# yijingru/KG_Instance_Segmentation

Measured on AMD Instinct MI355X. Metric: imgs/s (train fwd+bwd) at 512x512, higher is better.
Workload: dtype forward: f32-tolerance, hi + lo f16 planes (22 significant bits), 3 MFMA products / backward: f16 single planes, 1 MFMA product; f16 MFMA, fp32 accumulate; 1 GPU; KGnet train step fwd(dec+seg)+4xDetectionLossAll+SEG_loss+bwd+Adam, batch 8/GPU 3x512x512, 300 boxes/img, full HIP path; precision_policy=fp32, global_batch=8, parallelism=dp1, loss_readback=every step (train.py:156), grad_overflow=False

## Files before the change

### include/kgnet_hip.h

```cpp
#ifndef KGNET_HIP_H
#define KGNET_HIP_H
#ifdef __cplusplus
extern "C" {
#endif

typedef struct kg_planes {
    int a_planes, a_pstride;
    int b_planes, b_pstride;
    int c_planes, c_pstride;
    int y_planes, y_pstride;
    int w_planes;
    int reserved_;
    const float* scale;
    const float* oscale;
} kg_planes_t;

int kg_rows_format(void);

const char* kg_last_error(void);
const char* kg_last_kernel(void);
int kg_version(void);
int kg_device_arch(char* out, int cap);
int kg_tr_probe(void* out_u16x256, void* stream);
int kg_f64_probe(const double* a, const double* b, double* out5n, int n, void* stream);
// ... 26 lines not shown
int kg_pack_weight_batch(const void* jobs, int njobs, int total_blocks, void* stream);
int kg_im2col_small(const void* x, void* out, int N, int H, int W, int OH, int OW, int KH, int KW, int stride, int pad, int cin,
                    int ldx, int Kpad, void* stream);
int kg_conv2d_wgrad(const void* x, const void* dy, float* dwp, const int* rowdesc, int M, int H, int W, int OH, int OW,
                    int ldx, int lddy, int Cin, int Cout, int cin_lim, int cout_lim, int KH, int KW, int stride, int pad,
                    int dil, int mode, int nsplit, long split_stride, const kg_planes_t* planes, void* stream);
int kg_conv2d_wgrad_halo(const void* x, const void* dy, float* dwp, int N, int H, int W, int ldx, int lddy, int Cin, int Cout,
                         int cin_lim, int cout_lim, int KS, int nsplit, long split_stride, const int* tiletab16, int ntiles,
                         float* dbp, const kg_planes_t* planes, void* stream);
int kg_bias_grad_final(const float* part, float* db, int nsplit, int C, int accumulate, void* stream);
int kg_wgrad_reduce(const float* part, float* grad_oihw, int Cout, int Cin, int KH, int KW, int nsplit, long split_stride,
                    int accumulate, void* stream);
int kg_wgrad_reduce_multi(const float* part, float* const* grads_oihw, const int* counts, int ngrads, int Cin, int KH, int KW,
                          int nsplit, long split_stride, int accumulate, void* stream);
int kg_wgrad_reduce_bias(const float* part, float* const* grads_oihw, const int* counts, int ngrads, int Cin, int KH, int KW,
                         int nsplit, long split_stride, int accumulate, const float* bias_part, float* db, int bias_C, void* stream);
int kg_wgrad_reduce_defer(int on);
int kg_wgrad_reduce_pending(void);
int kg_wgrad_reduce_flush(void* stream);
int kg_bias_grad(const void* dy, float* db, float* scratch, int scratch_floats, int M, int C, int ld, int accumulate,
                 void* stream);
int kg_set_wgrad_tr(int use_transpose_read);

int kg_img_pack(const float* img_nchw, void* out_rows8, int ldout, int N, int C, int H, int W, const kg_planes_t* planes, void* stream);
int kg_bn_stats_train(const void* x, int ldx, int M, int C, const float* gamma, const float* beta, float* running_mean,
                      float* running_var, float momentum, float eps, float* mean_out, float* invstd_out, float* scale,
                      float* shift, float* scratch, int scratch_floats, const kg_planes_t* planes, void* stream);
int kg_conv_stats_begin(float* part, long cap_floats);
int kg_conv_stats_end(int* nb);
int kg_bn_finalize_train(const float* part, int nb, int M, int C, const float* gamma, const float* beta, float* running_mean,
                         float* running_var, float momentum, float eps, float* mean_out, float* invstd_out, float* scale,
                         float* shift, void* stream);
int kg_bn_scale_shift_eval(int C, const float* gamma, const float* beta, const float* running_mean,
                           const float* running_var, float eps, float* scale, float* shift, void* stream);
int kg_bn_apply(const void* x, int ldx, const float* scale, const float* shift, const void* res, int ldres, void* y,
                int ldy, int M, int C, int relu, const kg_planes_t* planes, void* stream);
int kg_bn_bwd(const void* x, int ldx, const void* dy, int lddy, const float* gamma, const float* mean,
              const float* invstd, float* dgamma, float* dbeta, int accumulate, void* dx, int lddx, int M, int C,
              float* scratch, int scratch_floats, const float* parts, int nb_parts, const float* parts_scale,
              const kg_planes_t* planes, void* stream);
int kg_bn_bwd_frozen(const void* x, int ldx, const void* dy, int lddy, const float* scale, const float* running_mean,
                     const float* running_var, float eps, float* dgamma, float* dbeta, int accumulate, void* dx, int lddx,
                     int M, int C, float* scratch, int scratch_floats, const kg_planes_t* planes, void* stream);
int kg_conv_bstats_begin(float* part, long cap_floats, const void* x, int ldx, int x_planes, int x_pstride, const float* mean,
                         const float* invstd);
int kg_maxpool3s2_fwd(const void* x, int ldx, void* y, int ldy, void* argmax_u8, int N, int H, int W, int C, const kg_planes_t* planes, void* stream);
int kg_maxpool3s2_bwd(const void* x, int ldx, const void* dy, int lddy, void* dx, int lddx, const void* argmax_u8, int N, int H, int W, int C,
                      const kg_planes_t* planes, void* stream);
int kg_bilinear_fwd(const void* x, int ldx, void* y, int ldy, int N, int IH, int IW, int OH, int OW, int C,
                    const int* boxdesc, const int* row2box, long total_out_rows, const kg_planes_t* planes, void* stream);
int kg_bilinear_bwd(const void* dy, int lddy, void* dx, int lddx, int N, int IH, int IW, int OH, int OW, int C,
                    const int* boxdesc, const int* row2box, long total_in_rows, const void* mask, int ldmask,
                    const kg_planes_t* planes, void* stream);
int kg_add_rows(const void* a, int lda, const void* b, int ldb, const void* mask, int ldm, void* y, int ldy, long M,
                int C, const float* scale, const float* scale2, const kg_planes_t* planes, void* stream);
int kg_sigmoid_inplace(float* x, long n, void* stream);
int kg_grad_pack(const float* g_nchw, const float* prob, void* out_rows, int N, int C, int H, int W, int ld, int cpad,
                 const kg_planes_t* planes, void* stream);
int kg_grad_pack3(const float* g0_nchw, const float* g1_nchw, const float* g2_nchw, const float* prob0, void* out_rows, int N, int C0, int C1, int C2,
                  int H, int W, int ld, int pad0, int pad1, int pad2, const kg_planes_t* planes, void* stream);

int kg_detection_loss_fwd(const float* kp, const float* sh, const float* md, const float* gt, int N, int H, int W,
                          float kp_radius, const float* den_override, float* scratch, int scratch_floats, float* out8,
                          void* stream);
int kg_detection_loss_bwd(const float* kp, const float* sh, const float* md, const float* gt, int N, int H, int W,
                          float kp_radius, const float* fin8, const float* grad_out, float* g_kp, float* g_sh,
                          float* g_md, void* stream);
int kg_seg_loss(const float* prob, const void* tgt_u8, const int* patches, const void* pairs, int npatches, float* part,
                float* out1, const float* grad_out, float* gprob, void* stream);

int kg_postproc_timing_begin(void);
int kg_postproc_timing_end(float* ms4);
long kg_postproc_workspace_bytes(int H, int W, int peak_cap, int skel_cap);
int kg_postproc_scale(const float* kp, const float* soff, const float* mid, int H, int W, double thresh, void* ws,
                      long ws_bytes, int peak_cap, int skel_cap, double* skel, int* nskel, double* heat_out,
                      double* blur_out, int* peaks_out, double* peak_conf_out, int* npeaks_out, void* stream);
int kg_skeleton_boxes(const double* skel, const int* nskel, int skel_cap, double scale, int do_refine, double* boxes,
                      int* nbox, int box_cap, void* stream);
int kg_nms(const double* boxes, const int* nbox, int box_cap, double thresh, void* ws, long ws_bytes, double* out,
           int* nkeep, void* stream);

long kg_postproc_batch_workspace_bytes(int N, int H, int W, int peak_cap, int skel_cap);
int kg_postproc_batch(const float* kp, const float* soff, const float* mid, int N, int H, int W, double thresh, void* ws,
                      long ws_bytes, int peak_cap, int skel_cap, double* skel, int* nskel, void* stream);
int kg_skeleton_boxes_batch(int N, int nscales, const double* const* skel, const int* const* nskel, const int* skel_cap,
                            const double* scale, int do_refine, double* boxes, int* nbox, int box_cap, void* stream);
long kg_nms_batch_workspace_bytes(int N, int box_cap);
int kg_nms_batch(int N, const double* boxes, const int* nbox, int box_cap, double thresh, void* ws, long ws_bytes, double* out,
                 int* nkeep, void* stream);

int kg_gt_maps(const float* kps, int n, int H, int W, float* out, void* stream);

int kg_sp_image(const void* imgs, int N, int H, int W, float* out, void* stream);
int kg_sp_warp_masks(const void* imgs, const int* inst_img, int ntot, int H, int W, void* out, int* box, void* stream);
int kg_sp_boxes(const void* imgs, int N, const int* box, int ntot, int kp_radius, int* counts, float* gtb, float* kp, int* keep,
                void* stream);

int kg_adam_step(const void* jobs, int njobs, int total_blocks, float beta1, float beta2, float eps, float step_size, float bc2_sqrt,
                 float weight_decay, void* stream);

int kg_host_crop_masks(const float* const* masks, const int* work, int nwork, int H, int W, unsigned char* out);
int kg_crop_masks(const void* masks, const int* work, int nwork, int H, int W, void* out, void* stream);
int kg_host_tile_table(const int* h, const int* w, const long* row0, int nb, int th, int tw, int* out, int cap);
int kg_host_bin_csr(const int* tab, int nb, int BS, int BY, int BX, int nbins, int* bin_start, int* bin_boxes, int cap);
int kg_host_match_boxes(const float* pb, int P, const float* gb, int G, int gstride, float thresh, int* pairs, int cap, int* count);

// ... 91 lines not shown
```

### kg_instance_segmentation_amd/_lib.py

```python
import ctypes
import os

_HERE = os.path.dirname(os.path.abspath(__file__))
LIB_PATH = os.environ.get("KG_LIB_PATH") or os.path.join(_HERE, "libkgnet_hip.so")
LIB_F16_PATH = os.environ.get("KG_LIB_F16_PATH") or os.path.join(os.path.dirname(LIB_PATH), "libkgnet_hip_f16.so")

c_int, c_long, c_float, c_double, c_void_p = ctypes.c_int, ctypes.c_long, ctypes.c_float, ctypes.c_double, ctypes.c_void_p
P = c_void_p

_SIGS = {
    "kg_version": [],
    "kg_rows_format": [],
    "kg_grad_scale": [P, P, P, c_int, c_int, P, P, P],
    "kg_scale_tensors": [P, c_int, c_int, P, P],
    "kg_rows_rescale": [P, c_int, c_long, c_int, c_int, P, P, P, P, P, P],
    "kg_rows_scale": [P, c_int, c_long, c_int, P, P, P, P],
    "kg_rows_scale_multi": [P, c_int, P, P, P],
    "kg_device_arch": [ctypes.c_char_p, c_int],
    "kg_tr_probe": [P, P],
    "kg_conv2d_igemm": [P, P, P, P, P, P, P, P] + [c_int] * 21 + [P, P],
    "kg_conv2d_halo": [P, P, P, P, P, P, P] + [c_int] * 15 + [P, c_int, c_int, P, P],
    "kg_conv1x1": [P, P, P, P, P, P, c_long] + [c_int] * 8 + [P],
    "kg_conv3x3_c64": [P, P, P, P, P, P] + [c_int] * 11 + [P, c_int, P],
    "kg_conv3x3_ws": [P, P, P, P] + [c_int] * 7 + [P, c_int, P, P],
    "kg_pack_weight": [P, P] + [c_int] * 11 + [P],
    "kg_pack_weight_rows": [P, P] + [c_int] * 6 + [P, c_int, c_int, c_int, c_int, P],
    "kg_pack_weight_batch": [P, c_int, c_int, P],
    "kg_pack_weight_narrow": [P, P] + [c_int] * 9 + [P],
    "kg_conv7_narrow": [P, P, P, P] + [c_int] * 11 + [P],
    "kg_im2col_small": [P, P] + [c_int] * 12 + [P],
    "kg_conv2d_halo_heads2": [P, P, P, P, P, P, P] + [c_int] * 7 + [P, P],
    "kg_set_wgrad_tr": [c_int],
    "kg_conv2d_wgrad": [P, P, P, P] + [c_int] * 18 + [c_long, P, P],
    "kg_conv2d_wgrad_halo": [P, P, P] + [c_int] * 11 + [c_long, P, c_int, P, P, P],
    "kg_bias_grad_final": [P, P, c_int, c_int, c_int, P],
    "kg_wgrad_reduce": [P, P, c_int, c_int, c_int, c_int, c_int, c_long, c_int, P],
    "kg_wgrad_reduce_multi": [P, P, P, c_int, c_int, c_int, c_int, c_int, c_long, c_int, P],
    "kg_wgrad_reduce_bias": [P, P, P, c_int, c_int, c_int, c_int, c_int, c_long, c_int, P, P, c_int, P],
    "kg_wgrad_reduce_defer": [c_int],
    "kg_wgrad_reduce_pending": [],
    "kg_wgrad_reduce_flush": [P],
    "kg_bias_grad": [P, P, P, c_int, c_int, c_int, c_int, c_int, P],
    "kg_img_pack": [P, P, c_int, c_int, c_int, c_int, c_int, P, P],
    "kg_bn_stats_train": [P, c_int, c_int, c_int, P, P, P, P, c_float, c_float, P, P, P, P, P, c_int, P, P],
    "kg_bn_scale_shift_eval": [c_int, P, P, P, P, c_float, P, P, P],
    "kg_conv_stats_begin": [P, c_long],
    "kg_conv_bstats_begin": [P, c_long, P, c_int, c_int, c_int, P, P],
    "kg_conv_stats_end": [P],
    "kg_bn_finalize_train": [P, c_int, c_int, c_int, P, P, P, P, c_float, c_float, P, P, P, P, P],
    "kg_bn_apply": [P, c_int, P, P, P, c_int, P, c_int, c_int, c_int, c_int, P, P],
    "kg_bn_bwd": [P, c_int, P, c_int, P, P, P, P, P, c_int, P, c_int, c_int, c_int, P, c_int, P, c_int, P, P, P],
    "kg_bn_bwd_frozen": [P, c_int, P, c_int, P, P, P, c_float, P, P, c_int, P, c_int, c_int, c_int, P, c_int, P, P],
    "kg_maxpool3s2_fwd": [P, c_int, P, c_int, P, c_int, c_int, c_int, c_int, P, P],
    "kg_maxpool3s2_bwd": [P, c_int, P, c_int, P, c_int, P, c_int, c_int, c_int, c_int, P, P],
    "kg_bilinear_fwd": [P, c_int, P, c_int, c_int, c_int, c_int, c_int, c_int, c_int, P, P, c_long, P, P],
    "kg_bilinear_bwd": [P, c_int, P, c_int, c_int, c_int, c_int, c_int, c_int, c_int, P, P, c_long, P, c_int, P, P],
    "kg_add_rows": [P, c_int, P, c_int, P, c_int, P, c_int, c_long, c_int, P, P, P, P],
    "kg_detection_loss_fwd": [P, P, P, P, c_int, c_int, c_int, c_float, P, P, c_int, P, P],
    "kg_detection_loss_bwd": [P, P, P, P, c_int, c_int, c_int, c_float, P, P, P, P, P, P],
    "kg_seg_loss": [P, P, P, P, c_int, P, P, P, P, P],
    "kg_sigmoid_inplace": [P, c_long, P],
    "kg_grad_pack": [P, P, P, c_int, c_int, c_int, c_int, c_int, c_int, P, P],
    "kg_grad_pack3": [P, P, P, P, P] + [c_int] * 10 + [P, P],
    "kg_postproc_workspace_bytes": [c_int, c_int, c_int, c_int],
    "kg_postproc_scale": [P, P, P, c_int, c_int, c_double, P, c_long, c_int, c_int, P, P, P, P, P, P, P, P],
    "kg_postproc_timing_begin": [],
    "kg_postproc_timing_end": [P],
    "kg_skeleton_boxes": [P, P, c_int, c_double, c_int, P, P, c_int, P],
    "kg_nms": [P, P, c_int, c_double, P, c_long, P, P, P],
    "kg_postproc_batch_workspace_bytes": [c_int, c_int, c_int, c_int, c_int],
    "kg_postproc_batch": [P, P, P, c_int, c_int, c_int, c_double, P, c_long, c_int, c_int, P, P, P],
    "kg_skeleton_boxes_batch": [c_int, c_int, P, P, P, P, c_int, P, P, c_int, P],
    "kg_nms_batch_workspace_bytes": [c_int, c_int],
    "kg_nms_batch": [c_int, P, P, c_int, c_double, P, c_long, P, P, P],
    "kg_gt_maps": [P, c_int, c_int, c_int, P, P],
    "kg_sp_image": [P, c_int, c_int, c_int, P, P],
    "kg_sp_warp_masks": [P, P, c_int, c_int, c_int, P, P, P],
    "kg_sp_boxes": [P, c_int, P, c_int, c_int, P, P, P, P, P],
    "kg_adam_step": [P, c_int, c_int, c_float, c_float, c_float, c_float, c_float, c_float, P],
    "kg_host_crop_masks": [P, P, c_int, c_int, c_int, P],
    "kg_crop_masks": [P, P, c_int, c_int, c_int, P, P],
    "kg_host_match_boxes": [P, c_int, P, c_int, c_int, c_float, P, c_int, P],
    "kg_host_tile_table": [P, P, P, c_int, c_int, c_int, P, c_int],
    "kg_host_bin_csr": [P, c_int, c_int, c_int, c_int, c_int, P, P, c_int],
    "kg_mask_areas": [P, c_int, c_long, P, P],
    "kg_mask_inter_pairs": [P, P, P, c_int, c_long, P, P],
    "kg_mask_bits_ld": [c_int, c_int],
    "kg_mask_pack_bits": [P, c_int, c_int, c_int, c_int, P, c_long, P],
    "kg_mask_unpack_bits": [P, c_long, c_int, c_int, c_int, P, c_int, P],
    "kg_bitmask_areas": [P, c_int, c_long, P, P],
    "kg_bitmask_inter_pairs": [P, c_int, P, c_int, P, c_int, c_long, P, P],
    "kg_instance_labels": [P, c_long, c_int, P, c_int, c_int, c_int, P, P, P, P],
    "kg_instance_overlay": [P, P, c_long, c_int, P, c_int, c_int, c_int, P, c_double, P, P],
    "kg_tile_cut": [P, c_int, c_int, P, c_int, P, c_int, c_int, c_int, P, P],
    "kg_bitmask_clip": [P, c_long, c_int, c_int, c_int, c_int, c_int, P],
    "kg_tile_stitch": [P, P, c_int, P, c_int, c_int, c_int, c_int, c_int, P, P],
    "kg_label_table": [P, c_int, c_int, P, c_int, P, P, P],
    "kg_label_stats": [P, c_int, c_int, c_int, P, P, P],
    "kg_label_inter_jobs": [P, P, c_int, c_int, P, c_int, P, P],
    "kg_label_components_workspace_bytes": [c_int, c_int, c_int],
    "kg_label_components": [P, c_int, c_int, c_int, c_int, c_int, P, P, P, c_long, P],
    "kg_component_stats": [P, P, c_int, c_int, c_int, P, c_int, P, P],
    "kg_component_remap": [P, c_int, c_int, c_int, P, c_int, P, P, P],
    "kg_label_measure": [P, c_int, c_int, c_int, P, c_int, c_int, P, c_int, P, P],
    "kg_label_distance": [P, c_int, c_int, c_int, c_int, c_int, P, P, P],
    "kg_label_regrow": [P, c_int, c_int, c_int, c_int, c_int, c_int, c_int, c_int, P, P],
    "kg_label_inscribed": [P, P, c_int, c_int, c_int, P, c_int, P, P],
    "kg_label_neighbours": [P, c_int, c_int, c_int, c_int, P, c_int, c_int, P, P],
    "kg_label_run_counts": [P, c_int, c_int, c_int, P, c_int, P, P],
# ... 99 lines not shown
```

### kg_instance_segmentation_amd/csrc/norm_pool.hip

```cpp
#include "kg_common.h"

struct RowsR { const bf16_t* p; int ld, P, ps; };
struct RowsW { bf16_t* p; int ld, P, ps; };
__device__ __forceinline__ void rd8(const RowsR& t, long r, int c, float (&v)[8]) { kg_load_planes8(t.p + r * t.ld + c, t.P, t.ps, v); }
__device__ __forceinline__ void wr8(const RowsW& t, long r, int c, float (&v)[8]) { kg_store_planes<8>(t.p + r * t.ld + c, t.P, t.ps, v, true); }
#define KG_PLANES(pl)                                                       \
    const kg_planes_t pp = kg_planes_or_default(pl);                        \
    KG_CHECK_ARG(kg_planes_ok(pp), "bad kg_planes_t (at most 3 planes, strides multiples of 8)")

__global__ void img_pack_kernel(const float* __restrict__ img, RowsW out, int N, int C, int HW) {
    long total = (long)N * HW;
    for (long i = blockIdx.x * (long)blockDim.x + threadIdx.x; i < total; i += (long)gridDim.x * blockDim.x) {
        long n = i / HW, p = i - n * HW;
        float v[8];
#pragma unroll
        for (int c = 0; c < 8; ++c) v[c] = c < C ? img[(n * C + c) * HW + p] : 0.f;
        wr8(out, i, 0, v);
    }
}
extern "C" int kg_img_pack(const float* img, void* out, int ldout, int N, int C, int H, int W, const kg_planes_t* planes, void* stream) {
    KG_CHECK_ARG(img && out && C <= 8 && ldout >= 8 && ldout % 8 == 0, "kg_img_pack: bad args");
    KG_PLANES(planes);
    long total = (long)N * H * W;
    int blocks = (int)((total + 255) / 256); if (blocks > 8192) blocks = 8192;
// ... 382 lines not shown
                int kw = ix - (ox * 2 - 1);
                if (kw < 0 || kw > 2) continue;
                float best[8]; int arg[8];
                if (argin) {
                    const uint2 pk = *reinterpret_cast<const uint2*>(argin + ((n * OH + oy) * OW + ox) * (long)(C8 * 8) + c);
#pragma unroll
                    for (int e = 0; e < 4; ++e) { arg[e] = (pk.x >> (8 * e)) & 255; arg[4 + e] = (pk.y >> (8 * e)) & 255; }
                } else
                    pool_window_max(x, n * H * W, H, W, oy, ox, c, best, arg);
                float ds[8];
                rd8(dy, (n * OH + oy) * OW + ox, c, ds);
#pragma unroll
                for (int e = 0; e < 8; ++e)
                    if (arg[e] == kh * 3 + kw) g[e] += ds[e];
            }
        }
        wr8(dx, p, c, g);
    }
}
extern "C" int kg_maxpool3s2_fwd(const void* x, int ldx, void* y, int ldy, void* argmax, int N, int H, int W, int C, const kg_planes_t* planes, void* stream) {
    KG_CHECK_ARG(x && y && C % 8 == 0 && ldx % 8 == 0 && ldy % 8 == 0, "kg_maxpool3s2_fwd: bad args");
    KG_PLANES(planes);
    int OH = (H + 2 - 3) / 2 + 1, OW = (W + 2 - 3) / 2 + 1;
    long total = (long)N * OH * OW * (C / 8);
    int blocks = (int)((total + 255) / 256); if (blocks > 16384) blocks = 16384;
    hipLaunchKernelGGL(maxpool_fwd_kernel, dim3(blocks), dim3(256), 0, (hipStream_t)stream, RowsR{(const bf16_t*)x, ldx, pp.a_planes, pp.a_pstride},
                       RowsW{(bf16_t*)y, ldy, pp.y_planes, pp.y_pstride}, (unsigned char*)argmax, N, H, W, OH, OW, C / 8);
    KG_CHECK_LAUNCH("maxpool_fwd");
    return KG_OK;
}
extern "C" int kg_maxpool3s2_bwd(const void* x, int ldx, const void* dy, int lddy, void* dx, int lddx, const void* argmax, int N, int H,
                                 int W, int C, const kg_planes_t* planes, void* stream) {
    KG_CHECK_ARG(x && dy && dx && C % 8 == 0 && ldx % 8 == 0 && lddy % 8 == 0 && lddx % 8 == 0, "kg_maxpool3s2_bwd: bad args");
    KG_PLANES(planes);
    int OH = (H + 2 - 3) / 2 + 1, OW = (W + 2 - 3) / 2 + 1;
    long total = (long)N * H * W * (C / 8);
    int blocks = (int)((total + 255) / 256); if (blocks > 16384) blocks = 16384;
    hipLaunchKernelGGL(maxpool_bwd_kernel, dim3(blocks), dim3(256), 0, (hipStream_t)stream, RowsR{(const bf16_t*)x, ldx, pp.a_planes, pp.a_pstride},
                       RowsR{(const bf16_t*)dy, lddy, pp.b_planes, pp.b_pstride}, (const unsigned char*)argmax, RowsW{(bf16_t*)dx, lddx, pp.y_planes, pp.y_pstride}, N, H, W, OH, OW, C / 8);
    KG_CHECK_LAUNCH("maxpool_bwd");
    return KG_OK;
}

__device__ __forceinline__ void bil_src(int dst, float scale, int in, int* i0, int* i1, float* l1) {
    float s = scale * ((float)dst + 0.5f) - 0.5f;
    if (s < 0.f) s = 0.f;
    int a = (int)s;
    if (a > in - 1) a = in - 1;
    *i0 = a; *i1 = a + (a < in - 1 ? 1 : 0); *l1 = s - (float)a;
}
__device__ __forceinline__ float bil_mix(float w00, float w01, float w10, float w11, float a, float b, float d, float e) {
    return __builtin_fmaf(w11, e, __builtin_fmaf(w10, d, __builtin_fmaf(w01, b, w00 * a)));
}
struct BilBox { int in_row0, ih, iw, out_row0, oh, ow; };
__global__ void bilinear_fwd_kernel(const RowsR x, const RowsW y, int IH,
                                    int IW, int OH, int OW, int C8, long total_rows, const BilBox* __restrict__ desc,
                                    const int* __restrict__ row2box) {
    long total = total_rows * C8;
    for (long i = blockIdx.x * (long)blockDim.x + threadIdx.x; i < total; i += (long)gridDim.x * blockDim.x) {
        long p; int c; kg_divmod(i, C8, &p, &c); c *= 8;
        long in0; int ih, iw, oh, ow, oy, ox;
        if (desc) {
            BilBox b = desc[row2box[p]];
            int loc = (int)(p - b.out_row0);
            ih = b.ih; iw = b.iw; oh = b.oh; ow = b.ow; oy = loc / ow; ox = loc - oy * ow; in0 = b.in_row0;
        } else {
            ih = IH; iw = IW; oh = OH; ow = OW;
            long q, nimg; kg_divmod(p, OW, &q, &ox); kg_divmod(q, OH, &nimg, &oy); in0 = nimg * IH * IW;
        }
        int y0, y1, x0, x1; float ly, lx;
        bil_src(oy, (float)ih / (float)oh, ih, &y0, &y1, &ly);
        bil_src(ox, (float)iw / (float)ow, iw, &x0, &x1, &lx);
        float w00 = (1.f - ly) * (1.f - lx), w01 = (1.f - ly) * lx, w10 = ly * (1.f - lx), w11 = ly * lx;
        float pa[8], pb[8], pd[8], pe[8];
        rd8(x, in0 + (long)y0 * iw + x0, c, pa); rd8(x, in0 + (long)y0 * iw + x1, c, pb);
        rd8(x, in0 + (long)y1 * iw + x0, c, pd); rd8(x, in0 + (long)y1 * iw + x1, c, pe);
        float v[8];
#pragma unroll
        for (int e = 0; e < 8; ++e) v[e] = bil_mix(w00, w01, w10, w11, pa[e], pb[e], pd[e], pe[e]);
        wr8(y, p, c, v);
    }
}
constexpr int BIL2_ROWS = 8;
__global__ __launch_bounds__(256) void bilinear2x_fwd_kernel(const RowsR x, const RowsW y, int N, int IH, int IW, int C8) {
    const long per_img = (long)IW * C8;
    const int strips = (IH + BIL2_ROWS - 1) / BIL2_ROWS;
    const long total = (long)N * strips * per_img;
    const int OH = 2 * IH, OW = 2 * IW;
    for (long t = blockIdx.x * (long)blockDim.x + threadIdx.x; t < total; t += (long)gridDim.x * blockDim.x) {
        long q; int c; kg_divmod(t, C8, &q, &c); c *= 8;
        int j; long q2; kg_divmod(q, IW, &q2, &j);
        int strip; long n; kg_divmod(q2, strips, &n, &strip);
        const int i0 = strip * BIL2_ROWS, i1 = i0 + BIL2_ROWS < IH ? i0 + BIL2_ROWS : IH;
        const long in0 = n * IH * IW, out0 = n * OH * OW;
        const int jl = j > 0 ? j - 1 : 0, jr = j < IW - 1 ? j + 1 : IW - 1;
        const float lx0 = j == 0 ? 0.f : 0.75f;
        float prev[3][8], cur[3][8], next[3][8];
        {
            const long bp = in0 + (long)(i0 > 0 ? i0 - 1 : 0) * IW, bc = in0 + (long)i0 * IW;
            rd8(x, bp + jl, c, prev[0]); rd8(x, bp + j, c, prev[1]); rd8(x, bp + jr, c, prev[2]);
            rd8(x, bc + jl, c, cur[0]); rd8(x, bc + j, c, cur[1]); rd8(x, bc + jr, c, cur[2]);
        }
        auto mix = [&](const float (&pa)[8], const float (&pb)[8], const float (&pd)[8], const float (&pe)[8], float ly, float lx, long orow) {
            const float w00 = (1.f - ly) * (1.f - lx), w01 = (1.f - ly) * lx, w10 = ly * (1.f - lx), w11 = ly * lx;
            float v[8];
#pragma unroll
            for (int e = 0; e < 8; ++e) v[e] = bil_mix(w00, w01, w10, w11, pa[e], pb[e], pd[e], pe[e]);
            wr8(y, orow, c, v);
        };
        for (int i = i0; i < i1; ++i) {
            const long bn = in0 + (long)(i < IH - 1 ? i + 1 : IH - 1) * IW;
            rd8(x, bn + jl, c, next[0]); rd8(x, bn + j, c, next[1]); rd8(x, bn + jr, c, next[2]);
            const float ly0 = i == 0 ? 0.f : 0.75f;
            const long o0 = out0 + (long)(2 * i) * OW + 2 * j, o1 = o0 + OW;
            mix(prev[0], prev[1], cur[0], cur[1], ly0, lx0, o0);
            mix(prev[1], prev[2], cur[1], cur[2], ly0, 0.25f, o0 + 1);
            mix(cur[0], cur[1], next[0], next[1], 0.25f, lx0, o1);
            mix(cur[1], cur[2], next[1], next[2], 0.25f, 0.25f, o1 + 1);
#pragma unroll
            for (int k = 0; k < 3; ++k)
#pragma unroll
                for (int e = 0; e < 8; ++e) { prev[k][e] = cur[k][e]; cur[k][e] = next[k][e]; }
        }
    }
}
__device__ __forceinline__ void bil_cand(int i, float scale, int out, int* lo, int* hi) {
    float a = ((float)i - 0.5f) / scale - 0.5f, b = ((float)i + 1.5f) / scale - 0.5f;
    int l = (int)floorf(a) - 1, h = (int)ceilf(b) + 1;
    *lo = l < 0 ? 0 : l; *hi = h > out - 1 ? out - 1 : h;
}
__global__ void bilinear_bwd_kernel(const RowsR dy, const RowsW dx, int IH,
                                    int IW, int OH, int OW, int C8, long total_rows, const BilBox* __restrict__ desc,
                                    const int* __restrict__ row2box, const bf16_t* __restrict__ mask, int ldmask) {
    long total = total_rows * C8;
    for (long i = blockIdx.x * (long)blockDim.x + threadIdx.x; i < total; i += (long)gridDim.x * blockDim.x) {
        long p; int c; kg_divmod(i, C8, &p, &c); c *= 8;
        long out0; int ih, iw, oh, ow, iy, ix;
        if (desc) {
            BilBox b = desc[row2box[p]];
            int loc = (int)(p - b.in_row0);
            ih = b.ih; iw = b.iw; oh = b.oh; ow = b.ow; iy = loc / iw; ix = loc - iy * iw; out0 = b.out_row0;
        } else {
            ih = IH; iw = IW; oh = OH; ow = OW;
            long q, nimg; kg_divmod(p, IW, &q, &ix); kg_divmod(q, IH, &nimg, &iy); out0 = nimg * OH * OW;
        }
        const float sy = (float)ih / (float)oh, sx = (float)iw / (float)ow;
        int ylo, yhi, xlo, xhi;
        bil_cand(iy, sy, oh, &ylo, &yhi); bil_cand(ix, sx, ow, &xlo, &xhi);
        float g[8];
#pragma unroll
        for (int e = 0; e < 8; ++e) g[e] = 0.f;
        for (int oy = ylo; oy <= yhi; ++oy) {
            int y0, y1; float ly;
            bil_src(oy, sy, ih, &y0, &y1, &ly);
            float wy = (y0 == iy ? 1.f - ly : 0.f) + (y1 == iy ? ly : 0.f);
            if (y0 != iy && y1 != iy) continue;
            for (int ox = xlo; ox <= xhi; ++ox) {
                int x0, x1; float lx;
                bil_src(ox, sx, iw, &x0, &x1, &lx);
                if (x0 != ix && x1 != ix) continue;
                float wx = (x0 == ix ? 1.f - lx : 0.f) + (x1 == ix ? lx : 0.f);
                float w = wy * wx;
                float ds[8];
                rd8(dy, out0 + (long)oy * ow + ox, c, ds);
#pragma unroll
                for (int e = 0; e < 8; ++e) g[e] += w * ds[e];
            }
        }
        if (mask) {
            const uint4 mv = *reinterpret_cast<const uint4*>(mask + p * ldmask + c);
            const bf16_t* ms = reinterpret_cast<const bf16_t*>(&mv);
#pragma unroll
            for (int e = 0; e < 8; ++e) g[e] = bf2f(ms[e]) > 0.f ? g[e] : 0.f;
        }
        wr8(dx, p, c, g);
    }
}
extern "C" int kg_bilinear_fwd(const void* x, int ldx, void* y, int ldy, int N, int IH, int IW, int OH, int OW, int C,
                               const int* boxdesc, const int* row2box, long total_out_rows, const kg_planes_t* planes, void* stream) {
    KG_CHECK_ARG(x && y && C % 8 == 0 && ldx % 8 == 0 && ldy % 8 == 0, "kg_bilinear_fwd: bad args");
    KG_PLANES(planes);
    long rows = boxdesc ? total_out_rows : (long)N * OH * OW;
    if (rows == 0) return KG_OK;
    long total = rows * (C / 8);
    static const int fast2x = getenv("KG_BILINEAR_2X") ? atoi(getenv("KG_BILINEAR_2X")) : 1;
    if (fast2x && !boxdesc && OH == 2 * IH && OW == 2 * IW && IH >= 2 && IW >= 2) {
        const long threads = (long)N * ((IH + BIL2_ROWS - 1) / BIL2_ROWS) * IW * (C / 8);
        int blocks2 = (int)((threads + 255) / 256); if (blocks2 > 65536) blocks2 = 65536;
        hipLaunchKernelGGL(bilinear2x_fwd_kernel, dim3(blocks2), dim3(256), 0, (hipStream_t)stream, RowsR{(const bf16_t*)x, ldx, pp.a_planes, pp.a_pstride},
                           RowsW{(bf16_t*)y, ldy, pp.y_planes, pp.y_pstride}, N, IH, IW, C / 8);
        KG_CHECK_LAUNCH("bilinear2x_fwd");
        return KG_OK;
    }
    int blocks = (int)((total + 255) / 256); if (blocks > 16384) blocks = 16384;
    hipLaunchKernelGGL(bilinear_fwd_kernel, dim3(blocks), dim3(256), 0, (hipStream_t)stream, RowsR{(const bf16_t*)x, ldx, pp.a_planes, pp.a_pstride},
                       RowsW{(bf16_t*)y, ldy, pp.y_planes, pp.y_pstride}, IH, IW, OH, OW, C / 8, rows, (const BilBox*)boxdesc, row2box);
    KG_CHECK_LAUNCH("bilinear_fwd");
    return KG_OK;
}
extern "C" int kg_bilinear_bwd(const void* dy, int lddy, void* dx, int lddx, int N, int IH, int IW, int OH, int OW, int C,
                               const int* boxdesc, const int* row2box, long total_in_rows, const void* mask, int ldmask,
                               const kg_planes_t* planes, void* stream) {
    KG_CHECK_ARG(dy && dx && C % 8 == 0 && lddy % 8 == 0 && lddx % 8 == 0 && (!mask || ldmask % 8 == 0), "kg_bilinear_bwd: bad args");
    KG_PLANES(planes);
    long rows = boxdesc ? total_in_rows : (long)N * IH * IW;
    if (rows == 0) return KG_OK;
    long total = rows * (C / 8);
    int blocks = (int)((total + 255) / 256); if (blocks > 16384) blocks = 16384;
    hipLaunchKernelGGL(bilinear_bwd_kernel, dim3(blocks), dim3(256), 0, (hipStream_t)stream, RowsR{(const bf16_t*)dy, lddy, pp.a_planes, pp.a_pstride},
                       RowsW{(bf16_t*)dx, lddx, pp.y_planes, pp.y_pstride}, IH, IW, OH, OW, C / 8, rows, (const BilBox*)boxdesc, row2box, (const bf16_t*)mask, ldmask);
    KG_CHECK_LAUNCH("bilinear_bwd");
    return KG_OK;
}

__global__ void add_rows_kernel(const RowsR a, const RowsR b,
                                const bf16_t* __restrict__ m, int ldm, const RowsW y, long M, int C8, const float* __restrict__ sc,
                                const float* __restrict__ sc2) {
    long total = M * C8;
    const float s = sc ? *sc * (sc2 ? *sc2 : 1.f) : 1.f;
    for (long i = blockIdx.x * (long)blockDim.x + threadIdx.x; i < total; i += (long)gridDim.x * blockDim.x) {
        long r; int c; kg_divmod(i, C8, &r, &c); c *= 8;
        float v[8];
        rd8(a, r, c, v);
        if (b.p) {
            float bs[8];
            rd8(b, r, c, bs);
#pragma unroll
            for (int e = 0; e < 8; ++e) v[e] += bs[e];
        }
        if (s != 1.f) {
#pragma unroll
            for (int e = 0; e < 8; ++e) v[e] *= s;
        }
        if (m) {
            uint4 mv = *reinterpret_cast<const uint4*>(m + r * ldm + c);
            const bf16_t* ms = (const bf16_t*)&mv;
#pragma unroll
            for (int e = 0; e < 8; ++e) v[e] = bf2f(ms[e]) > 0.f ? v[e] : 0.f;
        }
        wr8(y, r, c, v);
    }
}
extern "C" int kg_add_rows(const void* a, int lda, const void* b, int ldb, const void* mask, int ldm, void* y, int ldy,
                           long M, int C, const float* scale, const float* scale2, const kg_planes_t* planes, void* stream) {
    KG_PLANES(planes);
    KG_CHECK_ARG(a && y && C % 8 == 0 && lda % 8 == 0 && ldy % 8 == 0 && (!b || ldb % 8 == 0) && (!mask || ldm % 8 == 0), "kg_add_rows: bad args");
    if (M == 0) return KG_OK;
    long total = M * (C / 8);
    int blocks = (int)((total + 255) / 256); if (blocks > 16384) blocks = 16384;
    hipLaunchKernelGGL(add_rows_kernel, dim3(blocks), dim3(256), 0, (hipStream_t)stream, RowsR{(const bf16_t*)a, lda, pp.a_planes, pp.a_pstride},
                       RowsR{(const bf16_t*)b, ldb, pp.b_planes, pp.b_pstride}, (const bf16_t*)mask, ldm, RowsW{(bf16_t*)y, ldy, pp.y_planes, pp.y_pstride}, M, C / 8, scale, scale2);
    KG_CHECK_LAUNCH("add_rows");
    return KG_OK;
}

__global__ __launch_bounds__(1024) void rows_absmax_kernel(const RowsR g, long M, int C8, int target_log2, const float* __restrict__ cum_in,
                                                          float* __restrict__ cum_out, float* __restrict__ r_out, unsigned* scratch) {
    const long total = M * C8;
    unsigned best = 0;
    const long stride = (long)gridDim.x * blockDim.x;
    const long dr = stride / C8; const int dc = (int)(stride - dr * C8);
    long i = blockIdx.x * (long)blockDim.x + threadIdx.x;
    long r = i / C8; int c = (int)(i - r * C8);
// ... 133 lines not shown
```

### kg_instance_segmentation_amd/ops.py

```python
import functools
import math
import os

import torch

from . import _lib
from ._lib import c_int, c_long, c_float, c_double, ptr, stream_ptr

BF16 = torch.bfloat16
F16 = torch.float16
_scratch = {}
PARAM_EPOCH = [0]


def scratch_f32(nfloats, dev, tag="default"):
    key = (str(dev), tag)
    t = _scratch.get(key)
    if t is None or t.numel() < nfloats:
        t = torch.empty(max(int(nfloats), 1 << 16), dtype=torch.float32, device=dev)
        _scratch[key] = t
    return t


class WgradReduceQueue:
# ... 635 lines not shown
              ptr(st[0]), ptr(st[1]), ptr(st[2]), ptr(st[3]), stream_ptr())
    return st[0], st[1], st[2], st[3]


def bn_scale_shift_eval(C, gamma, beta, rmean, rvar, eps=1e-5):
    st = torch.empty(2, C, dtype=torch.float32, device=gamma.device)
    _lib.call("kg_bn_scale_shift_eval", C, ptr(gamma), ptr(beta), ptr(rmean), ptr(rvar), c_float(eps), ptr(st[0]), ptr(st[1]), stream_ptr())
    return st[0], st[1]


def bn_apply(x, C, scale, shift, y, res=None, relu=False):
    _lib.call("kg_bn_apply", ptr(_rows(x)), ld(x), ptr(scale), ptr(shift), ptr(base(res)), ld(res) if res is not None else 0, ptr(_rows(y)), ld(y),
              base(x).shape[0], C, 1 if relu else 0, pl(a=x, b=res, y=y), stream_ptr(), fmt=fmt_of(x))


def bn_bwd(x, dy, C, gamma, mean, invstd, dgamma, dbeta, dx, accumulate=False, parts=None, parts_scale=None):
    sc = scratch_f32(2 * C * 512 + 3 * C, base(x).device, "bn")
    pt, nbp = parts if parts is not None else (None, 0)
    _lib.call("kg_bn_bwd", ptr(_rows(x)), ld(x), ptr(_rows(dy)), ld(dy), ptr(gamma), ptr(mean), ptr(invstd), ptr(dgamma), ptr(dbeta),
              1 if accumulate else 0, ptr(_rows(dx)), ld(dx), base(x).shape[0], C, ptr(sc), sc.numel(), ptr(pt), nbp, ptr(parts_scale),
              pl(a=x, b=dy, y=dx), stream_ptr(), fmt=fmt_of(x))


def bn_bwd_frozen(x, dy, C, scale, rmean, rvar, dgamma, dbeta, dx, accumulate=False, eps=1e-5):
    if (dgamma is None) != (dbeta is None):
        raise ValueError("bn_bwd_frozen: dgamma and dbeta come together")
    sc = scratch_f32(2 * C * 512 + 3 * C, base(dy).device, "bn") if dgamma is not None else None
    _lib.call("kg_bn_bwd_frozen", ptr(base(x)), ld(x) if x is not None else 0, ptr(_rows(dy)), ld(dy), ptr(scale), ptr(rmean), ptr(rvar),
              c_float(eps), ptr(dgamma), ptr(dbeta), 1 if accumulate else 0, ptr(_rows(dx)), ld(dx), base(dy).shape[0], C, ptr(sc),
              sc.numel() if sc is not None else 0, pl(a=x, b=dy, y=dx), stream_ptr(), fmt=fmt_of(dy))


def maxpool_fwd(x, y, N, H, W, C, argmax=None):
    _lib.call("kg_maxpool3s2_fwd", ptr(_rows(x)), ld(x), ptr(_rows(y)), ld(y), ptr(argmax), N, H, W, C, pl(a=x, y=y), stream_ptr(), fmt=fmt_of(x))


def maxpool_bwd(x, dy, dx, N, H, W, C, argmax=None):
    _lib.call("kg_maxpool3s2_bwd", ptr(_rows(x)), ld(x), ptr(_rows(dy)), ld(dy), ptr(_rows(dx)), ld(dx), ptr(argmax), N, H, W, C,
              pl(a=x, b=dy, y=dx), stream_ptr(), fmt=fmt_of(dy))


def bilinear_fwd(x, y, N, IH, IW, OH, OW, C, boxdesc=None, row2box=None):
    rows = base(y).shape[0] if boxdesc is not None else 0
    _lib.call("kg_bilinear_fwd", ptr(_rows(x)), ld(x), ptr(_rows(y)), ld(y), N, IH, IW, OH, OW, C, ptr(boxdesc), ptr(row2box),
              c_long(rows), pl(a=x, y=y), stream_ptr(), fmt=fmt_of(x))


def bilinear_bwd(dy, dx, N, IH, IW, OH, OW, C, boxdesc=None, row2box=None, mask=None):
    rows = base(dx).shape[0] if boxdesc is not None else 0
    _lib.call("kg_bilinear_bwd", ptr(_rows(dy)), ld(dy), ptr(_rows(dx)), ld(dx), N, IH, IW, OH, OW, C, ptr(boxdesc), ptr(row2box),
              c_long(rows), ptr(base(mask)), ld(mask) if mask is not None else 0, pl(a=dy, y=dx), stream_ptr(), fmt=fmt_of(dy))


def add_rows(a, b, y, C, mask=None, scale=None):
    r, r2 = scale if scale is not None else (None, None)
    _lib.call("kg_add_rows", ptr(_rows(a)), ld(a), ptr(base(b)), ld(b) if b is not None else 0, ptr(base(mask)),
              ld(mask) if mask is not None else 0, ptr(_rows(y)), ld(y), c_long(base(a).shape[0]), C, ptr(r), ptr(r2), pl(a=a, b=b, y=y), stream_ptr(),
              fmt=fmt_of(a))


def planes_to_f32(x, C, out):
    _lib.call("kg_planes_to_f32", ptr(_rows(x)), ld(x), ptr(out), out.stride(0), c_long(base(x).shape[0]), C, pl(a=x), stream_ptr(), fmt=fmt_of(x))


def f32_to_planes(acc, y, C, addto=None, scale=None):
    _lib.call("kg_f32_to_planes", ptr(acc), acc.stride(0), ptr(_rows(y)), ld(y), ptr(base(addto)), ld(addto) if addto is not None else 0,
              c_long(acc.shape[0]), C, pl(b=addto, y=y, scale=scale), stream_ptr(), fmt=fmt_of(y))


def sigmoid_(x):
    _lib.call("kg_sigmoid_inplace", ptr(x), c_long(x.numel()), stream_ptr())
    return x


def grad_pack(g, prob, out, N, C, H, W, cpad, scale=None):
    _lib.call("kg_grad_pack", ptr(g), ptr(prob), ptr(_rows(out)), N, C, H, W, ld(out), cpad, pl(y=out, scale=scale), stream_ptr(), fmt=fmt_of(out))


def grad_pack3(gs, prob0, out, N, Cs, H, W, pads, scale=None):
    _lib.call("kg_grad_pack3", ptr(gs[0]), ptr(gs[1]), ptr(gs[2]), ptr(prob0), ptr(_rows(out)), N, Cs[0], Cs[1], Cs[2], H, W, ld(out),
              pads[0], pads[1], pads[2], pl(y=out, scale=scale), stream_ptr(), fmt=fmt_of(out))


GRAD_TARGET_LOG2 = int(__import__("os").environ.get("KG_GRAD_TARGET_LOG2", "4"))
_gs_state = {}


def grad_scale(tensors, probs=None):
    import ctypes
    probs = probs or [None] * len(tensors)
    pairs = [(t, q) for t, q in zip(tensors, probs) if t is not None and t.numel() > 0]
    ts = [t for t, _ in pairs]
    qs = [q for _, q in pairs]
    assert 1 <= len(ts) <= 24 and all(t.dtype == torch.float32 and t.is_contiguous() for t in ts)
    assert all(q is None or (q.dtype == torch.float32 and q.is_contiguous() and q.numel() == t.numel()) for t, q in pairs)
    dev = ts[0].device
    scr = _gs_state.get(str(dev))
    if scr is None:
        scr = torch.zeros(2, dtype=torch.int32, device=dev)
        _gs_state[str(dev)] = scr
    out = torch.empty(2, dtype=torch.float32, device=dev)
    ptrs = (ctypes.c_void_p * len(ts))(*[t.data_ptr() for t in ts])
    prbs = (ctypes.c_void_p * len(ts))(*[q.data_ptr() if q is not None else None for q in qs])
    cnts = (ctypes.c_long * len(ts))(*[t.numel() for t in ts])
    _lib.call("kg_grad_scale", ptrs, prbs, cnts, len(ts), GRAD_TARGET_LOG2, ptr(scr), ptr(out), stream_ptr())
    return out
# ... 47 lines not shown
```

Measured before the change: 129.1 imgs/s.

## Add strip-tiled 2x bilinear backward kernel and plane-specialized raw loads

Adds a dedicated bilinear2x backward kernel in which each thread walks a strip of input rows and reuses loaded dy rows across iterations, instead of using the generic per-pixel gather. It also specializes the forward kernels on plane count with raw uint4 loads, issuing all loads before summing the planes. The aim is to cut redundant global loads and indexing overhead in the upsample stages of the decoder. The cost is more template instantiations, higher register pressure from the raw buffers, and a reference toggle kept for the generic path.

After: 129.9 imgs/s, median of 6. Within noise of the previous version (+0.7%).

```diff
diff --git a/include/kgnet_hip.h b/include/kgnet_hip.h
--- a/include/kgnet_hip.h
+++ b/include/kgnet_hip.h
@@ -102,6 +102,7 @@
 int kg_bilinear_bwd(const void* dy, int lddy, void* dx, int lddx, int N, int IH, int IW, int OH, int OW, int C,
                     const int* boxdesc, const int* row2box, long total_in_rows, const void* mask, int ldmask,
                     const kg_planes_t* planes, void* stream);
+int kg_set_bilinear_reference(int on);
 int kg_add_rows(const void* a, int lda, const void* b, int ldb, const void* mask, int ldm, void* y, int ldy, long M,
                 int C, const float* scale, const float* scale2, const kg_planes_t* planes, void* stream);
 int kg_sigmoid_inplace(float* x, long n, void* stream);
diff --git a/kg_instance_segmentation_amd/_lib.py b/kg_instance_segmentation_amd/_lib.py
--- a/kg_instance_segmentation_amd/_lib.py
+++ b/kg_instance_segmentation_amd/_lib.py
@@ -55,6 +55,7 @@
     "kg_maxpool3s2_bwd": [P, c_int, P, c_int, P, c_int, P, c_int, c_int, c_int, c_int, P, P],
     "kg_bilinear_fwd": [P, c_int, P, c_int, c_int, c_int, c_int, c_int, c_int, c_int, P, P, c_long, P, P],
     "kg_bilinear_bwd": [P, c_int, P, c_int, c_int, c_int, c_int, c_int, c_int, c_int, P, P, c_long, P, c_int, P, P],
+    "kg_set_bilinear_reference": [c_int],
     "kg_add_rows": [P, c_int, P, c_int, P, c_int, P, c_int, c_long, c_int, P, P, P, P],
     "kg_detection_loss_fwd": [P, P, P, P, c_int, c_int, c_int, c_float, P, P, c_int, P, P],
     "kg_detection_loss_bwd": [P, P, P, P, c_int, c_int, c_int, c_float, P, P, P, P, P, P],
diff --git a/kg_instance_segmentation_amd/csrc/norm_pool.hip b/kg_instance_segmentation_amd/csrc/norm_pool.hip
--- a/kg_instance_segmentation_amd/csrc/norm_pool.hip
+++ b/kg_instance_segmentation_amd/csrc/norm_pool.hip
@@ -458,7 +458,25 @@
 __device__ __forceinline__ float bil_mix(float w00, float w01, float w10, float w11, float a, float b, float d, float e) {
     return __builtin_fmaf(w11, e, __builtin_fmaf(w10, d, __builtin_fmaf(w01, b, w00 * a)));
 }
+template <int P>
+__device__ __forceinline__ void bil_ld_raw(const RowsR& t, long r, int c, uint4 (&q)[P]) {
+#pragma unroll
+    for (int p = 0; p < P; ++p) q[p] = *reinterpret_cast<const uint4*>(t.p + r * t.ld + c + (long)p * t.ps);
+}
+template <int P>
+__device__ __forceinline__ void bil_sum_raw(const uint4 (&q)[P], float (&v)[8]) {
+    const bf16_t* s = reinterpret_cast<const bf16_t*>(&q[P - 1]);
+#pragma unroll
+    for (int e = 0; e < 8; ++e) v[e] = bf2f(s[e]);
+#pragma unroll
+    for (int p = P - 2; p >= 0; --p) {
+        const bf16_t* s2 = reinterpret_cast<const bf16_t*>(&q[p]);
+#pragma unroll
+        for (int e = 0; e < 8; ++e) v[e] += bf2f(s2[e]);
+    }
+}
 struct BilBox { int in_row0, ih, iw, out_row0, oh, ow; };
+template <int P>
 __global__ void bilinear_fwd_kernel(const RowsR x, const RowsW y, int IH,
                                     int IW, int OH, int OW, int C8, long total_rows, const BilBox* __restrict__ desc,
                                     const int* __restrict__ row2box) {
@@ -479,8 +497,15 @@
         bil_src(ox, (float)iw / (float)ow, iw, &x0, &x1, &lx);
         float w00 = (1.f - ly) * (1.f - lx), w01 = (1.f - ly) * lx, w10 = ly * (1.f - lx), w11 = ly * lx;
         float pa[8], pb[8], pd[8], pe[8];
-        rd8(x, in0 + (long)y0 * iw + x0, c, pa); rd8(x, in0 + (long)y0 * iw + x1, c, pb);
-        rd8(x, in0 + (long)y1 * iw + x0, c, pd); rd8(x, in0 + (long)y1 * iw + x1, c, pe);
+        if constexpr (P > 0) {
+            uint4 q[4][P];
+            bil_ld_raw<P>(x, in0 + (long)y0 * iw + x0, c, q[0]); bil_ld_raw<P>(x, in0 + (long)y0 * iw + x1, c, q[1]);
+            bil_ld_raw<P>(x, in0 + (long)y1 * iw + x0, c, q[2]); bil_ld_raw<P>(x, in0 + (long)y1 * iw + x1, c, q[3]);
+            bil_sum_raw<P>(q[0], pa); bil_sum_raw<P>(q[1], pb); bil_sum_raw<P>(q[2], pd); bil_sum_raw<P>(q[3], pe);
+        } else {
+            rd8(x, in0 + (long)y0 * iw + x0, c, pa); rd8(x, in0 + (long)y0 * iw + x1, c, pb);
+            rd8(x, in0 + (long)y1 * iw + x0, c, pd); rd8(x, in0 + (long)y1 * iw + x1, c, pe);
+        }
         float v[8];
 #pragma unroll
         for (int e = 0; e < 8; ++e) v[e] = bil_mix(w00, w01, w10, w11, pa[e], pb[e], pd[e], pe[e]);
@@ -488,6 +513,7 @@
     }
 }
 constexpr int BIL2_ROWS = 8;
+template <int P>
 __global__ __launch_bounds__(256) void bilinear2x_fwd_kernel(const RowsR x, const RowsW y, int N, int IH, int IW, int C8) {
     const long per_img = (long)IW * C8;
     const int strips = (IH + BIL2_ROWS - 1) / BIL2_ROWS;
@@ -504,8 +530,11 @@
         float prev[3][8], cur[3][8], next[3][8];
         {
             const long bp = in0 + (long)(i0 > 0 ? i0 - 1 : 0) * IW, bc = in0 + (long)i0 * IW;
-            rd8(x, bp + jl, c, prev[0]); rd8(x, bp + j, c, prev[1]); rd8(x, bp + jr, c, prev[2]);
-            rd8(x, bc + jl, c, cur[0]); rd8(x, bc + j, c, cur[1]); rd8(x, bc + jr, c, cur[2]);
+            uint4 q[6][P];
+            bil_ld_raw<P>(x, bp + jl, c, q[0]); bil_ld_raw<P>(x, bp + j, c, q[1]); bil_ld_raw<P>(x, bp + jr, c, q[2]);
+            bil_ld_raw<P>(x, bc + jl, c, q[3]); bil_ld_raw<P>(x, bc + j, c, q[4]); bil_ld_raw<P>(x, bc + jr, c, q[5]);
+#pragma unroll
+            for (int k = 0; k < 3; ++k) { bil_sum_raw<P>(q[k], prev[k]); bil_sum_raw<P>(q[3 + k], cur[k]); }
         }
         auto mix = [&](const float (&pa)[8], const float (&pb)[8], const float (&pd)[8], const float (&pe)[8], float ly, float lx, long orow) {
             const float w00 = (1.f - ly) * (1.f - lx), w01 = (1.f - ly) * lx, w10 = ly * (1.f - lx), w11 = ly * lx;
@@ -516,7 +545,10 @@
         };
         for (int i = i0; i < i1; ++i) {
             const long bn = in0 + (long)(i < IH - 1 ? i + 1 : IH - 1) * IW;
-            rd8(x, bn + jl, c, next[0]); rd8(x, bn + j, c, next[1]); rd8(x, bn + jr, c, next[2]);
+            uint4 q[3][P];
+            bil_ld_raw<P>(x, bn + jl, c, q[0]); bil_ld_raw<P>(x, bn + j, c, q[1]); bil_ld_raw<P>(x, bn + jr, c, q[2]);
+#pragma unroll
+            for (int k = 0; k < 3; ++k) bil_sum_raw<P>(q[k], next[k]);
             const float ly0 = i == 0 ? 0.f : 0.75f;
             const long o0 = out0 + (long)(2 * i) * OW + 2 * j, o1 = o0 + OW;
             mix(prev[0], prev[1], cur[0], cur[1], ly0, lx0, o0);
@@ -582,6 +614,67 @@
         wr8(dx, p, c, g);
     }
 }
+__device__ __forceinline__ void bil_acc(float (&g)[8], float w, const float (&ds)[8]) {
+#pragma unroll
+    for (int e = 0; e < 8; ++e) g[e] = __builtin_fmaf(w, ds[e], g[e]);
+}
+__device__ __forceinline__ void bil_relu_mask(float (&g)[8], const uint4 mv) {
+    const bf16_t* ms = reinterpret_cast<const bf16_t*>(&mv);
+#pragma unroll
+    for (int e = 0; e < 8; ++e) g[e] = bf2f(ms[e]) > 0.f ? g[e] : 0.f;
+}
+template <int P>
+__global__ __launch_bounds__(256) void bilinear2x_bwd_kernel(const RowsR dy, const RowsW dx, int N, int IH, int IW, int C8,
+                                                             const bf16_t* __restrict__ mask, int ldmask) {
+    const long per_img = (long)IW * C8;
+    const int strips = (IH + BIL2_ROWS - 1) / BIL2_ROWS;
+    const long total = (long)N * strips * per_img;
+    const int OH = 2 * IH, OW = 2 * IW;
+    for (long t = blockIdx.x * (long)blockDim.x + threadIdx.x; t < total; t += (long)gridDim.x * blockDim.x) {
+        long q; int c; kg_divmod(t, C8, &q, &c); c *= 8;
+        int j; long q2; kg_divmod(q, IW, &q2, &j);
+        int strip; long n; kg_divmod(q2, strips, &n, &strip);
+        const int i0 = strip * BIL2_ROWS, i1 = i0 + BIL2_ROWS < IH ? i0 + BIL2_ROWS : IH;
+        const long in0 = n * IH * IW, out0 = n * OH * OW;
+        const int col[4] = {j > 0 ? 2 * j - 1 : 0, 2 * j, 2 * j + 1, j < IW - 1 ? 2 * j + 2 : OW - 1};
+        const float wx[4] = {j > 0 ? 0.25f : 0.f, j == 0 ? 1.f : 0.75f, j == IW - 1 ? 1.f : 0.75f, j < IW - 1 ? 0.25f : 0.f};
+        float a[2][4][8];
+        uint4 raw[2][4][P];
+        {
+            const long r0 = out0 + (long)(i0 > 0 ? 2 * i0 - 1 : 0) * OW, r1 = out0 + (long)(2 * i0) * OW;
+#pragma unroll
+            for (int k = 0; k < 4; ++k) { bil_ld_raw<P>(dy, r0 + col[k], c, raw[0][k]); bil_ld_raw<P>(dy, r1 + col[k], c, raw[1][k]); }
+#pragma unroll
+            for (int k = 0; k < 4; ++k) { bil_sum_raw<P>(raw[0][k], a[0][k]); bil_sum_raw<P>(raw[1][k], a[1][k]); }
+        }
+        for (int i = i0; i < i1; ++i) {
+            const long r2 = out0 + (long)(2 * i + 1) * OW, r3 = out0 + (long)(i < IH - 1 ? 2 * i + 2 : OH - 1) * OW;
+#pragma unroll
+            for (int k = 0; k < 4; ++k) { bil_ld_raw<P>(dy, r2 + col[k], c, raw[0][k]); bil_ld_raw<P>(dy, r3 + col[k], c, raw[1][k]); }
+            const long p = in0 + (long)i * IW + j;
+            uint4 mv = {0u, 0u, 0u, 0u};
+            if (mask) mv = *reinterpret_cast<const uint4*>(mask + p * ldmask + c);
+            const float wy[4] = {i > 0 ? 0.25f : 0.f, i == 0 ? 1.f : 0.75f, i == IH - 1 ? 1.f : 0.75f, i < IH - 1 ? 0.25f : 0.f};
+            float g[8];
+#pragma unroll
+            for (int e = 0; e < 8; ++e) g[e] = 0.f;
+#pragma unroll
+            for (int k = 0; k < 4; ++k) bil_acc(g, wy[0] * wx[k], a[0][k]);
+#pragma unroll
+            for (int k = 0; k < 4; ++k) bil_acc(g, wy[1] * wx[k], a[1][k]);
+#pragma unroll
+            for (int k = 0; k < 4; ++k) { bil_sum_raw<P>(raw[0][k], a[0][k]); bil_sum_raw<P>(raw[1][k], a[1][k]); }
+#pragma unroll
+            for (int k = 0; k < 4; ++k) bil_acc(g, wy[2] * wx[k], a[0][k]);
+#pragma unroll
+            for (int k = 0; k < 4; ++k) bil_acc(g, wy[3] * wx[k], a[1][k]);
+            if (mask) bil_relu_mask(g, mv);
+            wr8(dx, p, c, g);
+        }
+    }
+}
+static int g_bilinear_reference = 0;
+extern "C" int kg_set_bilinear_reference(int on) { g_bilinear_reference = on; return KG_OK; }
 extern "C" int kg_bilinear_fwd(const void* x, int ldx, void* y, int ldy, int N, int IH, int IW, int OH, int OW, int C,
                                const int* boxdesc, const int* row2box, long total_out_rows, const kg_planes_t* planes, void* stream) {
     KG_CHECK_ARG(x && y && C % 8 == 0 && ldx % 8 == 0 && ldy % 8 == 0, "kg_bilinear_fwd: bad args");
@@ -590,16 +683,18 @@
     if (rows == 0) return KG_OK;
     long total = rows * (C / 8);
     static const int fast2x = getenv("KG_BILINEAR_2X") ? atoi(getenv("KG_BILINEAR_2X")) : 1;
-    if (fast2x && !boxdesc && OH == 2 * IH && OW == 2 * IW && IH >= 2 && IW >= 2) {
+    if (fast2x && !g_bilinear_reference && !boxdesc && OH == 2 * IH && OW == 2 * IW && IH >= 2 && IW >= 2) {
         const long threads = (long)N * ((IH + BIL2_ROWS - 1) / BIL2_ROWS) * IW * (C / 8);
         int blocks2 = (int)((threads + 255) / 256); if (blocks2 > 65536) blocks2 = 65536;
-        hipLaunchKernelGGL(bilinear2x_fwd_kernel, dim3(blocks2), dim3(256), 0, (hipStream_t)stream, RowsR{(const bf16_t*)x, ldx, pp.a_planes, pp.a_pstride},
+        auto kern2 = pp.a_planes == 1 ? bilinear2x_fwd_kernel<1> : pp.a_planes == 2 ? bilinear2x_fwd_kernel<2> : bilinear2x_fwd_kernel<3>;
+        hipLaunchKernelGGL(kern2, dim3(blocks2), dim3(256), 0, (hipStream_t)stream, RowsR{(const bf16_t*)x, ldx, pp.a_planes, pp.a_pstride},
                            RowsW{(bf16_t*)y, ldy, pp.y_planes, pp.y_pstride}, N, IH, IW, C / 8);
         KG_CHECK_LAUNCH("bilinear2x_fwd");
         return KG_OK;
     }
     int blocks = (int)((total + 255) / 256); if (blocks > 16384) blocks = 16384;
-    hipLaunchKernelGGL(bilinear_fwd_kernel, dim3(blocks), dim3(256), 0, (hipStream_t)stream, RowsR{(const bf16_t*)x, ldx, pp.a_planes, pp.a_pstride},
+    auto kern = g_bilinear_reference ? bilinear_fwd_kernel<0> : pp.a_planes == 1 ? bilinear_fwd_kernel<1> : pp.a_planes == 2 ? bilinear_fwd_kernel<2> : bilinear_fwd_kernel<3>;
+    hipLaunchKernelGGL(kern, dim3(blocks), dim3(256), 0, (hipStream_t)stream, RowsR{(const bf16_t*)x, ldx, pp.a_planes, pp.a_pstride},
                        RowsW{(bf16_t*)y, ldy, pp.y_planes, pp.y_pstride}, IH, IW, OH, OW, C / 8, rows, (const BilBox*)boxdesc, row2box);
     KG_CHECK_LAUNCH("bilinear_fwd");
     return KG_OK;
@@ -612,9 +707,20 @@
     long rows = boxdesc ? total_in_rows : (long)N * IH * IW;
     if (rows == 0) return KG_OK;
     long total = rows * (C / 8);
+    const RowsR g{(const bf16_t*)dy, lddy, pp.a_planes, pp.a_pstride};
+    const RowsW o{(bf16_t*)dx, lddx, pp.y_planes, pp.y_pstride};
+    static const int fast2x = getenv("KG_BILINEAR_2X") ? atoi(getenv("KG_BILINEAR_2X")) : 1;
+    if (fast2x && !g_bilinear_reference && !boxdesc && OH == 2 * IH && OW == 2 * IW && IH >= 2 && IW >= 2) {
+        const long threads = (long)N * ((IH + BIL2_ROWS - 1) / BIL2_ROWS) * IW * (C / 8);
+        int blocks2 = (int)((threads + 255) / 256); if (blocks2 > 65536) blocks2 = 65536;
+        auto kern = pp.a_planes == 1 ? bilinear2x_bwd_kernel<1> : pp.a_planes == 2 ? bilinear2x_bwd_kernel<2> : bilinear2x_bwd_kernel<3>;
+        hipLaunchKernelGGL(kern, dim3(blocks2), dim3(256), 0, (hipStream_t)stream, g, o, N, IH, IW, C / 8, (const bf16_t*)mask, ldmask);
+        KG_CHECK_LAUNCH("bilinear2x_bwd");
+        return KG_OK;
+    }
     int blocks = (int)((total + 255) / 256); if (blocks > 16384) blocks = 16384;
-    hipLaunchKernelGGL(bilinear_bwd_kernel, dim3(blocks), dim3(256), 0, (hipStream_t)stream, RowsR{(const bf16_t*)dy, lddy, pp.a_planes, pp.a_pstride},
-                       RowsW{(bf16_t*)dx, lddx, pp.y_planes, pp.y_pstride}, IH, IW, OH, OW, C / 8, rows, (const BilBox*)boxdesc, row2box, (const bf16_t*)mask, ldmask);
+    hipLaunchKernelGGL(bilinear_bwd_kernel, dim3(blocks), dim3(256), 0, (hipStream_t)stream, g, o, IH, IW, OH, OW, C / 8, rows, (const BilBox*)boxdesc, row2box,
+                       (const bf16_t*)mask, ldmask);
     KG_CHECK_LAUNCH("bilinear_bwd");
     return KG_OK;
 }
diff --git a/kg_instance_segmentation_amd/ops.py b/kg_instance_segmentation_amd/ops.py
--- a/kg_instance_segmentation_amd/ops.py
+++ b/kg_instance_segmentation_amd/ops.py
@@ -711,6 +711,10 @@
               c_long(rows), ptr(base(mask)), ld(mask) if mask is not None else 0, pl(a=dy, y=dx), stream_ptr(), fmt=fmt_of(dy))
 
 
+def set_bilinear_reference(on, fmt=0):
+    _lib.call("kg_set_bilinear_reference", int(bool(on)), fmt=fmt)
+
+
 def add_rows(a, b, y, C, mask=None, scale=None):
     r, r2 = scale if scale is not None else (None, None)
     _lib.call("kg_add_rows", ptr(_rows(a)), ld(a), ptr(base(b)), ld(b) if b is not None else 0, ptr(base(mask)),
```
